# nico-bohlinger/RL-X

Measured on NVIDIA H100. Metric: env-steps/sec (PPO update incl.), higher is better.
Workload: dtype f32

## Files before the change

### rl_x_b200/csrc/gemm_tc.cu

```cuda
#include "gemm_dispatch.cuh"
#include "gemm_tc_common.cuh"

namespace rlx {
namespace tc {

struct Cfg {
  static constexpr int A_BYTES = BM * BK * 4;
  static constexpr int B_BYTES = BN * BK * 4;
  static constexpr int RAW_BYTES = A_BYTES + B_BYTES;
  static constexpr int OP_BYTES = 2 * B_BYTES;
  static constexpr int RAW_STAGES = 3, OP_STAGES = 4;
  static constexpr int SMEM_BYTES = RAW_STAGES * RAW_BYTES + OP_STAGES * OP_BYTES + 1024  + 1024 ;
  static constexpr int SPLIT_STAGE_BYTES = A_BYTES + 2 * B_BYTES;
  static constexpr int SPLIT_STAGES = 4;
  static constexpr int SPLIT_SMEM_BYTES = SPLIT_STAGES * SPLIT_STAGE_BYTES + 1024 + 1024;
  static constexpr int PRODUCER_REGS = 56, CONSUMER_REGS = 224;
};
static_assert(Cfg::SMEM_BYTES <= 227 * 1024 && Cfg::SPLIT_SMEM_BYTES <= 227 * 1024, "shared memory of one H100 block");
static_assert(Cfg::PRODUCER_REGS * 128 + Cfg::CONSUMER_REGS * 256 <= 65536, "register file of one SM");

template <bool KMAJ, bool BF16, int ROWS>
__device__ __forceinline__ void convert_tile(const uint8_t* raw, uint8_t* hi, uint8_t* lo, int t) {
  constexpr uint32_t HI = 0xFFFFE000u;
  if (KMAJ) {
// ... 178 lines not shown

  if (warp < 4) {
    setmaxnreg_dec<Cfg::PRODUCER_REGS>();
    const int t = threadIdx.x;
    uint64_t* ld_empty = SPLIT_B ? op_empty : raw_empty;
    int ld_tile = blockIdx.x, ld_kb = 0, ld_count = 0;
    auto load_next = [&]() {
      while (ld_tile < num_tiles) {
        int zb, zs, m0, n0, kbeg, nkb;
        tile_coords(ld_tile, zb, zs, m0, n0, kbeg, nkb);
        if (ld_kb >= nkb) {
          ld_tile += gridDim.x;
          ld_kb = 0;
          continue;
        }
        const int slot = ld_count % RAW_STAGES;
        mbar_wait(&ld_empty[slot], ((ld_count / RAW_STAGES) & 1) ^ 1);
        uint8_t* sa = smem + slot * RAW_BYTES;
        uint8_t* sb = sa + Cfg::A_BYTES;
        uint64_t* bar = &raw_full[slot];
        const int k0 = kbeg + ld_kb * BK;
        mbar_arrive_expect_tx(bar, RAW_BYTES);
        if (A_KMAJ) {
          tma_load_2d(&tmap_a, bar, sa, p.a_k_off * zb + k0, p.a_mn_off * zb + m0);
        } else {
#pragma unroll
          for (int j = 0; j < BM / 32; ++j) tma_load_2d(&tmap_a, bar, sa + j * (BK * 128), p.a_mn_off * zb + m0 + 32 * j, p.a_k_off * zb + k0);
        }
        if (B_KMAJ) {
          tma_load_2d(&tmap_b, bar, sb, p.b_k_off * zb + k0, p.b_mn_off * zb + n0);
          if (SPLIT_B) tma_load_2d(&tmap_b_lo, bar, sb + Cfg::B_BYTES, p.b_k_off * zb + k0, p.b_mn_off * zb + n0);
        } else {
#pragma unroll
          for (int j = 0; j < BN / 32; ++j) tma_load_2d(&tmap_b, bar, sb + j * (BK * 128), p.b_mn_off * zb + n0 + 32 * j, p.b_k_off * zb + k0);
        }
        ++ld_kb;
        ++ld_count;
        return true;
      }
      return false;
    };
    if constexpr (SPLIT_B) {
      if (t == 0)
        while (load_next()) {
        }
      return;
    }
    if (t == 0)
      for (int i = 0; i < RAW_STAGES; ++i) load_next();
    int rs = 0, os = 0;
    uint32_t rph = 0, oph = 0;
    bool refill = false;
    for (int tile = blockIdx.x; tile < num_tiles; tile += gridDim.x) {
      int zb, zs, m0, n0, kbeg, nkb;
      tile_coords(tile, zb, zs, m0, n0, kbeg, nkb);
      for (int kb = 0; kb < nkb; ++kb) {
        mbar_wait(&raw_full[rs], rph);
        mbar_wait(&op_empty[os], oph ^ 1);
        uint8_t* op = ops + os * Cfg::OP_BYTES;
        convert_tile<B_KMAJ, BF16, BN>(smem + rs * Cfg::RAW_BYTES + Cfg::A_BYTES, op, op + Cfg::B_BYTES, t);
        fence_proxy_async();
        named_bar_sync(1, 128);
        if (t == 0) {
          mbar_arrive(&op_full[os]);
          mbar_arrive(&raw_empty[rs]);
          if (refill) load_next();
          refill = true;
        }
        if (++rs == RAW_STAGES) { rs = 0; rph ^= 1; }
        if (++os == OP_STAGES) { os = 0; oph ^= 1; }
      }
    }
  } else {
    setmaxnreg_inc<Cfg::CONSUMER_REGS>();
    const int cw = (warp >> 2) - 1;
    const int r0 = cw * 64 + (warp & 3) * 16 + (lane >> 2);
    float acc[64], cor[64];
    uint32_t ah[2][2][4], al[2][2][4];
    int rs = 0, os = 0;
    uint32_t rph = 0, oph = 0;
    for (int tile = blockIdx.x; tile < num_tiles; tile += gridDim.x) {
      int zb, zs, m0, n0, kbeg, nkb;
      tile_coords(tile, zb, zs, m0, n0, kbeg, nkb);
      for (int kb = 0; kb < nkb; ++kb) {
        mbar_wait(&raw_full[rs], rph);
        if (!SPLIT_B) mbar_wait(&op_full[os], oph);
        const uint8_t* raw = smem + rs * RAW_BYTES;
        const uint32_t op = SPLIT_B ? smem_u32(raw + Cfg::A_BYTES) : smem_u32(ops + os * Cfg::OP_BYTES);
        const uint64_t db = make_smem_desc(op), db_lo = make_smem_desc(op + Cfg::B_BYTES);
#pragma unroll
        for (int h = 0; h < 2; ++h) {
          load_a_frags<A_KMAJ, BF16>(raw, r0, lane, h, ah[h], al[h]);
          if (!SPLIT_B && h == 1) {
            __syncwarp();
            if (lane == 0) mbar_arrive(&raw_empty[rs]);
          }
          fence_frags(ah[h]);
          if (!BF16) fence_frags(al[h]);
          wgmma_fence();
#pragma unroll
          for (int q = 0; q < 2; ++q) {
            const int kk = 2 * h + q;
            const uint64_t ko = (uint64_t)((kk * WG_K * 4) >> 4);
            const uint32_t accum = (kb | kk) != 0 ? 1u : 0u;
            if (!BF16) {
              wgmma_tf32_m64n128k8(cor, al[h][q], db + ko, accum);
              wgmma_tf32_m64n128k8(cor, ah[h][q], db_lo + ko, 1u);
            }
            wgmma_tf32_m64n128k8(acc, ah[h][q], db + ko, accum);
          }
          wgmma_commit();
          wgmma_wait_1();
          if (h == 0 && kb > 0 && lane == 0) mbar_arrive(&op_empty[os == 0 ? OP_STAGES - 1 : os - 1]);
        }
        if (++rs == RAW_STAGES) { rs = 0; rph ^= 1; }
        if (++os == OP_STAGES) { os = 0; oph ^= 1; }
      }

      constexpr bool HAS_AUX = (EPI == TC_EPI_DTANH || EPI == TC_EPI_DRELU);
      constexpr bool HAS_BIAS = (EPI == TC_EPI_BIAS_TANH || EPI == TC_EPI_BIAS_RELU || EPI == TC_EPI_BIAS);
      const int m = m0 + r0, ct = n0 + 2 * (lane & 3);
      const bool full = m0 + BM <= (TRANS ? p.m_main : p.M) && n0 + BN <= p.N;
      const int clim = p.N - 1 - ct;
      const float* abase = HAS_AUX ? p.aux + p.aux_batch_off * zb + ct : nullptr;
      float e[2][32];
      auto load_aux = [&](int q) {
        const float* arow = abase + (long long)min(m + 8 * (q >> 1), p.M - 1) * p.ldaux;
        if (full) load_cols<true>(e[q >> 1], arow, clim, 8 * (q & 1));
        else load_cols<false>(e[q >> 1], arow, clim, 8 * (q & 1));
      };
      if (HAS_BIAS) {
        const float* b = p.bias + p.bias_batch_off * zb + ct;
#pragma unroll
        for (int c0 = 0; c0 < 16; c0 += 8) {
          if (full) load_cols<true>(e[0], b, clim, c0);
          else load_cols<false>(e[0], b, clim, c0);
        }
      }
      if (HAS_AUX) load_aux(0);
      if (nkb > 0) {
        wgmma_wait_all();
        if (lane == 0) mbar_arrive(&op_empty[os == 0 ? OP_STAGES - 1 : os - 1]);
      }
      fence_acc(acc);
      if (!BF16) fence_acc(cor);
      float* cbase = p.C + p.c_batch_off * zb + p.c_split_off * zs;
      float* ebase = (TRANS && p.extra_row != nullptr) ? p.extra_row + p.extra_batch_off * zb + p.extra_split_off * zs : nullptr;
      if (full) store_tile<EPI, BF16, TRANS, true>(acc, cor, e, p, cbase, ebase, m, ct, load_aux);
      else store_tile<EPI, BF16, TRANS, false>(acc, cor, e, p, cbase, ebase, m, ct, load_aux);
    }
  }
}

template <bool A_KMAJ, bool B_KMAJ, int EPI, bool BF16 = false, bool TRANS = false, bool SPLIT_B = false>
static int launch_cfg(const TcOperand& A, const TcOperand& B, TcParams p, int kclass, cudaStream_t stream, const float* b_lo = nullptr) {
  CUtensorMap ta, tb, tb_lo;
  int rc = make_tmap(&ta, A.base, A.rows, A.cols, A.ld, 32, A_KMAJ ? BM : BK);
  if (rc) return rc;
  rc = make_tmap(&tb, B.base, B.rows, B.cols, B.ld, 32, B_KMAJ ? BN : BK);
  if (rc) return rc;
  if (SPLIT_B) {
    rc = make_tmap(&tb_lo, b_lo, B.rows, B.cols, B.ld, 32, BN);
    if (rc) return rc;
  } else {
    tb_lo = tb;
  }
// ... 167 lines not shown
```

### rl_x_b200/csrc/gemm_tc_common.cuh

```cuda
#pragma once
#include <cuda.h>

#include "common.cuh"
#include "gemm_simt.cuh"

namespace rlx {
namespace tc {

constexpr int BM = 128;
constexpr int BN = 128;
constexpr int BK = 32;
constexpr int WG_K = 8;
constexpr int NUM_THREADS = 384;

enum TcEpi { TC_EPI_NONE = 0, TC_EPI_BIAS_TANH = 1, TC_EPI_DTANH = 2, TC_EPI_BIAS_RELU = 3, TC_EPI_DRELU = 4, TC_EPI_BIAS = 5 };

struct TcParams {
  int M, N, K;
  int batch, splits, kchunk;
  int tiles_m, tiles_n;
  int a_mn_off, a_k_off, b_mn_off, b_k_off;
  float* C;
  long long ldc, c_batch_off, c_split_off;
  int m_main;
  float* extra_row;
  long long extra_batch_off, extra_split_off;
  const float* bias;
  long long bias_batch_off;
  const float* aux;
  long long ldaux, aux_batch_off;
  int single;
  int bf16;
};

__device__ __forceinline__ uint32_t smem_u32(const void* p) { return (uint32_t)__cvta_generic_to_shared(p); }

__device__ __forceinline__ void mbar_init(uint64_t* bar, uint32_t count) {
  asm volatile("mbarrier.init.shared::cta.b64 [%0], %1;" ::"r"(smem_u32(bar)), "r"(count) : "memory");
}
__device__ __forceinline__ void mbar_wait(uint64_t* bar, uint32_t parity) {
  asm volatile(
      "{\n\t"
      ".reg .pred P1;\n\t"
      "WAIT_LOOP:\n\t"
      "mbarrier.try_wait.parity.shared::cta.b64 P1, [%0], %1;\n\t"
      "@P1 bra WAIT_DONE;\n\t"
      "bra WAIT_LOOP;\n\t"
      "WAIT_DONE:\n\t"
      "}" ::"r"(smem_u32(bar)), "r"(parity)
      : "memory");
}
__device__ __forceinline__ void mbar_arrive(uint64_t* bar) {
  asm volatile("mbarrier.arrive.shared::cta.b64 _, [%0];" ::"r"(smem_u32(bar)) : "memory");
}
__device__ __forceinline__ void mbar_arrive_expect_tx(uint64_t* bar, uint32_t bytes) {
  asm volatile("mbarrier.arrive.expect_tx.shared::cta.b64 _, [%0], %1;" ::"r"(smem_u32(bar)), "r"(bytes) : "memory");
}
__device__ __forceinline__ void fence_barrier_init() { asm volatile("fence.mbarrier_init.release.cluster;" ::: "memory"); }
__device__ __forceinline__ void fence_proxy_async() { asm volatile("fence.proxy.async.shared::cta;" ::: "memory"); }
__device__ __forceinline__ void named_bar_sync(int id, int threads) { asm volatile("bar.sync %0, %1;" ::"r"(id), "r"(threads) : "memory"); }

__device__ __forceinline__ void tma_load_2d(const CUtensorMap* map, uint64_t* bar, void* smem, int c0, int c1) {
  asm volatile("cp.async.bulk.tensor.2d.shared::cluster.global.mbarrier::complete_tx::bytes [%0], [%1, {%3, %4}], [%2];" ::"r"(smem_u32(smem)),
               "l"((uint64_t)map), "r"(smem_u32(bar)), "r"(c0), "r"(c1)
               : "memory");
}
__device__ __forceinline__ void prefetch_tmap(const CUtensorMap* map) {
  asm volatile("prefetch.tensormap [%0];" ::"l"((uint64_t)map) : "memory");
}

__device__ __forceinline__ uint64_t make_smem_desc(uint32_t saddr) {
  uint64_t d = 0;
  d |= (uint64_t)((saddr >> 4) & 0x3FFFu);
  d |= (uint64_t)1u << 16;
  d |= (uint64_t)(1024u >> 4) << 32;
  d |= 1ull << 62;
  return d;
}

__device__ __forceinline__ void wgmma_fence() { asm volatile("wgmma.fence.sync.aligned;" ::: "memory"); }
__device__ __forceinline__ void wgmma_commit() { asm volatile("wgmma.commit_group.sync.aligned;" ::: "memory"); }
__device__ __forceinline__ void wgmma_wait_all() { asm volatile("wgmma.wait_group.sync.aligned 0;" ::: "memory"); }
__device__ __forceinline__ void wgmma_wait_1() { asm volatile("wgmma.wait_group.sync.aligned 1;" ::: "memory"); }
__device__ __forceinline__ void fence_acc(float (&d)[64]) {
#pragma unroll
  for (int i = 0; i < 64; ++i) asm volatile("" : "+f"(d[i])::"memory");
}
__device__ __forceinline__ void fence_frags(uint32_t (&a)[2][4]) {
#pragma unroll
  for (int i = 0; i < 2; ++i)
#pragma unroll
    for (int j = 0; j < 4; ++j) asm volatile("" : "+r"(a[i][j])::"memory");
}

template <int N> __device__ __forceinline__ void setmaxnreg_dec() { asm volatile("setmaxnreg.dec.sync.aligned.u32 %0;" ::"n"(N)); }
template <int N> __device__ __forceinline__ void setmaxnreg_inc() { asm volatile("setmaxnreg.inc.sync.aligned.u32 %0;" ::"n"(N)); }

__device__ __forceinline__ void wgmma_tf32_m64n128k8(float (&d)[64], const uint32_t (&a)[4], uint64_t b_desc, uint32_t accumulate) {
  asm volatile(
      "{\n\t"
      ".reg .pred p;\n\t"
      "setp.ne.b32 p, %69, 0;\n\t"
      "wgmma.mma_async.sync.aligned.m64n128k8.f32.tf32.tf32 "
      "{%0, %1, %2, %3, %4, %5, %6, %7, %8, %9, %10, %11, %12, %13, %14, %15, "
      "%16, %17, %18, %19, %20, %21, %22, %23, %24, %25, %26, %27, %28, %29, %30, %31, "
      "%32, %33, %34, %35, %36, %37, %38, %39, %40, %41, %42, %43, %44, %45, %46, %47, "
      "%48, %49, %50, %51, %52, %53, %54, %55, %56, %57, %58, %59, %60, %61, %62, %63}, "
      "{%64, %65, %66, %67}, %68, p, 1, 1;\n\t"
      "}"
      : "+f"(d[0]), "+f"(d[1]), "+f"(d[2]), "+f"(d[3]), "+f"(d[4]), "+f"(d[5]), "+f"(d[6]), "+f"(d[7]), "+f"(d[8]), "+f"(d[9]),
        "+f"(d[10]), "+f"(d[11]), "+f"(d[12]), "+f"(d[13]), "+f"(d[14]), "+f"(d[15]), "+f"(d[16]), "+f"(d[17]), "+f"(d[18]),
        "+f"(d[19]), "+f"(d[20]), "+f"(d[21]), "+f"(d[22]), "+f"(d[23]), "+f"(d[24]), "+f"(d[25]), "+f"(d[26]), "+f"(d[27]),
        "+f"(d[28]), "+f"(d[29]), "+f"(d[30]), "+f"(d[31]), "+f"(d[32]), "+f"(d[33]), "+f"(d[34]), "+f"(d[35]), "+f"(d[36]),
        "+f"(d[37]), "+f"(d[38]), "+f"(d[39]), "+f"(d[40]), "+f"(d[41]), "+f"(d[42]), "+f"(d[43]), "+f"(d[44]), "+f"(d[45]),
        "+f"(d[46]), "+f"(d[47]), "+f"(d[48]), "+f"(d[49]), "+f"(d[50]), "+f"(d[51]), "+f"(d[52]), "+f"(d[53]), "+f"(d[54]),
        "+f"(d[55]), "+f"(d[56]), "+f"(d[57]), "+f"(d[58]), "+f"(d[59]), "+f"(d[60]), "+f"(d[61]), "+f"(d[62]), "+f"(d[63])
      : "r"(a[0]), "r"(a[1]), "r"(a[2]), "r"(a[3]), "l"(b_desc), "r"(accumulate)
      : "memory");
}


typedef CUresult (*EncodeTiledFn)(CUtensorMap*, CUtensorMapDataType, cuuint32_t, void*, const cuuint64_t*, const cuuint64_t*, const cuuint32_t*,
                                  const cuuint32_t*, CUtensorMapInterleave, CUtensorMapSwizzle, CUtensorMapL2promotion, CUtensorMapFloatOOBfill);

static inline EncodeTiledFn get_encode_fn() {
  static EncodeTiledFn fn = nullptr;
  static bool tried = false;
  if (!tried) {
    tried = true;
    void* ptr = nullptr;
    cudaDriverEntryPointQueryResult q;
    if (cudaGetDriverEntryPoint("cuTensorMapEncodeTiled", &ptr, cudaEnableDefault, &q) == cudaSuccess && q == cudaDriverEntryPointSuccess)
      fn = reinterpret_cast<EncodeTiledFn>(ptr);
  }
  return fn;
}

static inline int make_tmap(CUtensorMap* map, const float* base, long long rows, long long cols, long long ld, int box_cols, int box_rows) {
  EncodeTiledFn fn = get_encode_fn();
  if (!fn) {
    set_error("tensor-core engine: cuTensorMapEncodeTiled is unavailable");
    return RLX_ERR_UNSUPPORTED;
  }
  cuuint64_t gdim[2] = {(cuuint64_t)cols, (cuuint64_t)rows};
  cuuint64_t gstride[1] = {(cuuint64_t)ld * 4};
  cuuint32_t box[2] = {(cuuint32_t)box_cols, (cuuint32_t)box_rows};
  cuuint32_t estr[2] = {1, 1};
// ... 18 lines not shown
```

### rl_x_b200/csrc/ppo.cu

```cuda
#include "common.cuh"
#include "gemm_simt.cuh"
#include "gemm_dispatch.cuh"
#include "ppo_head.cuh"
#include "ppo_head_gemm.cuh"
#include "ppo_head_mma.cuh"
#include "ppo_optim.cuh"

namespace rlx {

static bool use_tc(const rlx_ppo_dims& d) { return g_gemm_engine == 1 && tc_supported(d); }
}
int comm_allreduce_ppo(rlx_comm* c, float* out, int64_t n, const rlx_ppo_dims& d, float* norm_partials, long long* step_count, void* stream, int* nblk_out);
namespace rlx {

struct Splits {
  int splits, kchunk;
};
static Splits choose_splits(long long rows, int out_m, int out_n, int batch, bool tc) {
  if (tc) {
    const long long tiles = ceil_div(out_m, 128) * ceil_div(out_n, 128) * batch;
    const long long smin = std::max<long long>(1, ceil_div(rows, 1024)), smax = std::max<long long>(smin, std::min<long long>(smin + 64, rows / 64));
    const long long sms = sm_count();
    long long best = smin;
    double best_fill = -1.0;
// ... 262 lines not shown
}

static long long tall_elements(const GradReduceP& r) {
  long long tall = 0;
  for (int gi = 0; gi < kNumGroups; ++gi)
    if (r.g[gi].nsplit > kTallSplit) tall += r.g[gi].len;
  return tall;
}
static double partial_bytes(const GradReduceP& r) {
  double b = 0;
  for (int gi = 0; gi < kNumGroups; ++gi) b += 4.0 * r.g[gi].nsplit * r.g[gi].len;
  return b;
}
static int launch_grad_reduce(const GradReduceP& r, cudaStream_t st) {
  const int flat_blocks = (int)ceil_div(r.total, 256);
  const int tall_blocks = (int)ceil_div(tall_elements(r), 8);
  RLX_LAUNCH_C(KC_GRAD_REDUCE, 0, partial_bytes(r) + 4.0 * r.total, ppo_grad_reduce_kernel, (unsigned)(flat_blocks + tall_blocks), 256, 0, st, r, flat_blocks);
  return RLX_OK;
}

static bool fast_head_ok(const PpoLayout& L) { return (L.act <= 31) && (L.H % 2 == 0) && (L.H <= 1024); }

static int launch_train_head(const rlx_ppo_minibatch_args* a, const PpoLayout& L, const TrainPlan& P, const float* params, int bf16, cudaStream_t st) {
  const long long m = a->m;
  const int H = L.H, A = L.act;
  void* ws = a->workspace;
  float* H2 = ws_ptr<float>(ws, P.off_H2);
  float* dZ2 = ws_ptr<float>(ws, P.off_dZ2);
  float* dhead = ws_ptr<float>(ws, P.off_dhead);
  float* headpart = ws_ptr<float>(ws, P.off_headpart);
  const float inv_mg = 1.f / (float)a->m_global;
  HeadP h{};
  fill_head_common(h, L, params, H2, m);
  h.bf16 = bf16;
  h.actions = a->actions; h.logp_old = a->log_probs; h.adv = a->advantages; h.ret = a->returns; h.adv_stats = a->adv_stats;
  h.inv_mg = inv_mg; h.clip_range = a->hp.clip_range; h.critic_coef = a->hp.critic_coef;
  h.ratio_delta_metric = a->hp.ratio_delta_metric != 0.f ? 1 : 0;
  const bool want_median = a->hp.ratio_delta_metric == 2.f;
  h.ratio_abs = want_median ? ws_ptr<float>(ws, P.off_ratio) : nullptr;
  h.dZ2 = dZ2; h.dhead = dhead; h.block_partials = headpart;
  int head_blocks = P.head_blocks;
  const size_t smem = head_smem_bytes(a->dims, true);
  const int dh_ld = (int)(ceil_div(A + 1, 4) * 4);
  const bool fast_head = fast_head_ok(L);
  const double head_flops = 4.0 * m * H * (A + 1), head_bytes = 4.0 * m * (4.0 * H + 2.0 * A + 5);
  const bool gemm_head = fast_head && g_head_engine == 1 && !bf16 && head_gemm_scratch_floats(m, H, A) <= m * 2LL * H;
  if (gemm_head) {
    HeadGemmArgs ha{m, H, A, dh_ld, H2, a->params + L.off[W3P], a->params + L.off[W3C], a->params + L.off[B3P], a->params + L.off[B3C],
                    a->params + L.off[LOGSTD], a->actions, a->log_probs, a->advantages, a->returns, a->adv_stats, inv_mg, a->hp.clip_range,
                    a->hp.critic_coef, a->hp.ratio_delta_metric != 0.f ? 1 : 0, dZ2, dhead, headpart, ws_ptr<float>(ws, P.off_dZ1)};
    const int rc = ppo_head_gemm_path(ha, st);
    if (rc) return rc;
    return 1;
  }
  if (!fast_head) {
    RLX_DISPATCH_NCH(KC_HEAD_TRAIN, head_flops, head_bytes, H, ppo_head_train_kernel, head_blocks, 256, smem, st, h);
    return head_blocks;
  }
  HeadTrain2Extra ex{dh_ld};
  const bool vec_head = (H == 128 || H == 256 || H == 512);
  const int nt4 = (int)ceil_div(dh_ld, 8);
  const size_t smem4 = head4_smem_floats(H, A, nt4) * sizeof(float);
  const bool mma_head = vec_head && g_head_engine == 2 && !bf16 && nt4 <= 4 && smem4 <= 220 * 1024;
  if (mma_head) {
    head_blocks = (int)std::min<long long>(ceil_div(m, 16 * kHead4RowTiles), (long long)P.head_blocks);
#define RLX_HEAD4(H_, NT_)                                                                                                          \
  do {                                                                                                                              \
    RLX_CHECK_CUDA(cudaFuncSetAttribute(ppo_head_train4_kernel<H_, NT_>, cudaFuncAttributeMaxDynamicSharedMemorySize, (int)smem4)); \
    RLX_LAUNCH_C(KC_HEAD_TRAIN, head_flops, head_bytes, (ppo_head_train4_kernel<H_, NT_>), head_blocks, 256, smem4, st, h, ex);     \
  } while (0)
#define RLX_HEAD4_NT(H_)              \
  do {                                \
    if (nt4 == 1) RLX_HEAD4(H_, 1);   \
    else if (nt4 == 2) RLX_HEAD4(H_, 2); \
    else if (nt4 == 3) RLX_HEAD4(H_, 3); \
    else RLX_HEAD4(H_, 4);            \
  } while (0)
    if (H == 128) RLX_HEAD4_NT(128);
    else if (H == 256) RLX_HEAD4_NT(256);
    else RLX_HEAD4_NT(512);
#undef RLX_HEAD4_NT
#undef RLX_HEAD4
  } else if (vec_head) {
#define RLX_HEAD3_B(H_, AM_, BF_)                                                                                                     \
  do {                                                                                                                                \
    RLX_CHECK_CUDA(cudaFuncSetAttribute(ppo_head_train3_kernel<H_, AM_, BF_>, cudaFuncAttributeMaxDynamicSharedMemorySize, (int)smem)); \
    RLX_LAUNCH_C(KC_HEAD_TRAIN, head_flops, head_bytes, (ppo_head_train3_kernel<H_, AM_, BF_>), head_blocks, 256, smem, st, h, ex);    \
  } while (0)
#define RLX_HEAD3(H_, AM_)                          \
  do {                                              \
    if (bf16) RLX_HEAD3_B(H_, AM_, true);           \
    else RLX_HEAD3_B(H_, AM_, false);               \
  } while (0)
#define RLX_HEAD3_ACT(H_)                      \
  do {                                         \
    if (A <= 8) RLX_HEAD3(H_, 8);              \
    else if (A <= 16) RLX_HEAD3(H_, 16);       \
    else if (A <= 24) RLX_HEAD3(H_, 24);       \
    else RLX_HEAD3(H_, 31);                    \
  } while (0)
    if (H == 128) RLX_HEAD3_ACT(128);
    else if (H == 256) RLX_HEAD3_ACT(256);
    else RLX_HEAD3_ACT(512);
#undef RLX_HEAD3_ACT
#undef RLX_HEAD3
#undef RLX_HEAD3_B
  } else {
    const int nch = (int)ceil_div(H, 32);
#define RLX_HEAD2_B(NCH_, AM_, BF_)                                                                                                   \
  do {                                                                                                                                \
    RLX_CHECK_CUDA(cudaFuncSetAttribute(ppo_head_train2_kernel<NCH_, AM_, BF_>, cudaFuncAttributeMaxDynamicSharedMemorySize, (int)smem)); \
    RLX_LAUNCH_C(KC_HEAD_TRAIN, head_flops, head_bytes, (ppo_head_train2_kernel<NCH_, AM_, BF_>), head_blocks, 256, smem, st, h, ex);  \
  } while (0)
#define RLX_HEAD2(NCH_, AM_)                        \
  do {                                              \
    if (bf16) RLX_HEAD2_B(NCH_, AM_, true);         \
    else RLX_HEAD2_B(NCH_, AM_, false);             \
  } while (0)
#define RLX_HEAD2_ACT(NCH_)                         \
  do {                                              \
    if (A <= 8) RLX_HEAD2(NCH_, 8);                 \
    else if (A <= 16) RLX_HEAD2(NCH_, 16);          \
    else if (A <= 24) RLX_HEAD2(NCH_, 24);          \
    else RLX_HEAD2(NCH_, 31);                       \
  } while (0)
    if (nch <= 2) RLX_HEAD2_ACT(2);
    else if (nch <= 4) RLX_HEAD2_ACT(4);
    else if (nch <= 8) RLX_HEAD2_ACT(8);
    else if (nch <= 16) RLX_HEAD2_ACT(16);
    else RLX_HEAD2_ACT(32);
#undef RLX_HEAD2_ACT
#undef RLX_HEAD2
#undef RLX_HEAD2_B
  }
  return head_blocks;
}

struct W3Partials {
  float* src;
  int nsplit;
  long long stride, critic_off;
};
static W3Partials chunked_w3(const PpoLayout& L, float* part3, int nchunks) {
  return W3Partials{part3, nchunks, (long long)(L.act + 1) * L.H, (long long)L.act * L.H};
}

static int launch_head_wgrad(const PpoLayout& L, const TrainPlan& P, long long m, bool tc, int bf16, void* ws, cudaStream_t st, W3Partials& w3) {
  const int H = L.H, A = L.act;
  float* H2 = ws_ptr<float>(ws, P.off_H2);
  float* dhead = ws_ptr<float>(ws, P.off_dhead);
  float* part3 = ws_ptr<float>(ws, P.off_part3);
  const int wgrad_chunks = (int)ceil_div(m, kHeadWgradRows);
  const double wflops = 2.0 * m * H * (A + 1), wbytes = 4.0 * m * (2.0 * H + A + 1);
  if (!fast_head_ok(L)) {
    HeadWgradP w{(int)m, H, A, kHeadWgradRows, H2, dhead, part3};
    dim3 wg((unsigned)wgrad_chunks, (unsigned)ceil_div(2 * H, 256));
    const size_t wsmem = (size_t)kHeadWgradRows * (A + 1) * sizeof(float);
    if (A <= 8) RLX_LAUNCH_C(KC_HEAD_WGRAD, wflops, wbytes, ppo_head_wgrad_kernel<8>, wg, 256, wsmem, st, w);
    else if (A <= 32) RLX_LAUNCH_C(KC_HEAD_WGRAD, wflops, wbytes, ppo_head_wgrad_kernel<32>, wg, 256, wsmem, st, w);
    else {
      RLX_CHECK_CUDA(cudaFuncSetAttribute(ppo_head_wgrad_kernel<64>, cudaFuncAttributeMaxDynamicSharedMemorySize, (int)wsmem));
      RLX_LAUNCH_C(KC_HEAD_WGRAD, wflops, wbytes, ppo_head_wgrad_kernel<64>, wg, 256, wsmem, st, w);
    }
    count_gemm_path(GP_HEAD_WGRAD_SIMT);
    w3 = chunked_w3(L, part3, wgrad_chunks);
    return RLX_OK;
  }
  const int dh_ld = (int)(ceil_div(A + 1, 4) * 4);
  if (tc) {
    const Splits S3 = choose_splits(m, dh_ld, H, 2, true);
// ... 352 lines not shown
```

### rl_x_b200/csrc/ppo_head.cuh

```cuda
#pragma once
#include "common.cuh"

namespace rlx {

constexpr float kLogSqrt2Pi = 0.91893853320467274178f;

__device__ __forceinline__ void philox4x32_10(uint32_t (&c)[4], uint32_t k0, uint32_t k1) {
#pragma unroll
  for (int r = 0; r < 10; ++r) {
    const uint32_t hi0 = __umulhi(0xD2511F53u, c[0]), lo0 = 0xD2511F53u * c[0];
    const uint32_t hi1 = __umulhi(0xCD9E8D57u, c[2]), lo1 = 0xCD9E8D57u * c[2];
    const uint32_t n0 = hi1 ^ c[1] ^ k0, n1 = lo1, n2 = hi0 ^ c[3] ^ k1, n3 = lo0;
    c[0] = n0; c[1] = n1; c[2] = n2; c[3] = n3;
    k0 += 0x9E3779B9u; k1 += 0xBB67AE85u;
  }
}
__device__ __forceinline__ float philox_normal(uint64_t seed, uint64_t offset, uint32_t row, uint32_t j) {
  uint32_t c[4] = {row, j >> 2, (uint32_t)offset, (uint32_t)(offset >> 32)};
  philox4x32_10(c, (uint32_t)seed, (uint32_t)(seed >> 32));
  const uint32_t a = (j & 2) ? c[2] : c[0], b = (j & 2) ? c[3] : c[1];
  const float u1 = ((float)a + 0.5f) * 2.3283064365386963e-10f;
  const float u2 = ((float)b + 0.5f) * 2.3283064365386963e-10f;
  const float r = sqrtf(-2.f * logf(fminf(u1, 1.f)));
  float s, co;
  sincospif(2.f * u2, &s, &co);
  return (j & 1) ? r * s : r * co;
}

struct HeadP {
  int M, H, act;
  const float* H2;
  const float* W3p;
  const float* W3c;
  const float* b3p;
  const float* b3c;
  const float* logstd;
  const float* noise;
  unsigned long long seed, offset;
  const float* act_low;
  const float* act_high;
  int clip_rescale, deterministic;
  float* action;
  float* env_action;
  float* logp_out;
  float* value_out;
  const float* actions;
  const float* logp_old;
  const float* adv;
  const float* ret;
  const float* adv_stats;
  float inv_mg;
  float clip_range, critic_coef;
  int ratio_delta_metric;
  float* ratio_abs;
  float* dZ2;
  float* dhead;
  float* block_partials;
  int bf16;
};

template <int NCH, bool BF16>
__device__ __forceinline__ void head_row_forward(const HeadP& p, const float* __restrict__ sW3p, const float* __restrict__ sW3c,
                                                 long long row, int lane, float (&hp)[NCH], float (&hc)[NCH], float& mean_lo,
                                                 float& mean_hi, float& value) {
  const float* __restrict__ h = p.H2 + row * (2LL * p.H);
#pragma unroll
  for (int c = 0; c < NCH; ++c) {
    const int j = lane + 32 * c;
    hp[c] = (j < p.H) ? h[j] : 0.f;
    hc[c] = (j < p.H) ? h[p.H + j] : 0.f;
  }
  mean_lo = 0.f;
  mean_hi = 0.f;
  for (int a = 0; a < p.act; ++a) {
    float s = 0.f;
#pragma unroll
    for (int c = 0; c < NCH; ++c) {
      const int j = lane + 32 * c;
      if (j < p.H) s = fmaf(hp[c], sW3p[a * p.H + j], s);
    }
    s = bf16r_if(warp_sum(s) + p.b3p[a], BF16);
    if (lane == (a & 31)) {
      if (a < 32) mean_lo = s; else mean_hi = s;
    }
// ... 343 lines not shown
#pragma unroll
    for (int c = 0; c < NCH; ++c) dz0[c] = dz1[c] = 0.f;
#pragma unroll
    for (int a = 0; a < ACT_MAX; ++a) {
      if (a < act) {
        const float g0 = __shfl_sync(0xffffffffu, dmean[0], a);
        const float g1 = __shfl_sync(0xffffffffu, dmean[1], a);
#pragma unroll
        for (int c = 0; c < NCH; ++c) {
          const int j = lane + 32 * c;
          const float w = (j < H) ? sW3p[a * H + j] : 0.f;
          dz0[c] = fmaf(g0, w, dz0[c]);
          dz1[c] = fmaf(g1, w, dz1[c]);
        }
      }
    }
#pragma unroll
    for (int r = 0; r < 2; ++r) {
      if (r == 1 && !has1) break;
      float* __restrict__ out = p.dZ2 + (row0 + r) * (2LL * H);
#pragma unroll
      for (int c = 0; c < NCH; ++c) {
        const int j = lane + 32 * c;
        if (j < H) {
          const float hpv = hp[r][c], hcv = hc[r][c];
          const float zp = bf16r_if(bf16r_if(r ? dz1[c] : dz0[c], BF16) * (1.f - hpv * hpv), BF16);
          const float zc = bf16r_if(bf16r_if(dvv[r] * sW3c[j], BF16) * (1.f - hcv * hcv), BF16);
          out[j] = zp;
          out[H + j] = zc;
          acc_db2p[c] += zp;
          acc_db2c[c] += zc;
        }
      }
    }
  }

  float* my = sred + wib * npart;
  if (own) {
    my[lane] = acc_db3;
    my[act + 1 + lane] = acc_dls;
  } else if (lane == act) {
    my[act] = acc_db3;
  }
  if (lane == 0) {
    my[2 * act + 1] = acc_pg;
    my[2 * act + 2] = acc_vl;
    my[2 * act + 3] = acc_kl;
    my[2 * act + 4] = acc_cf;
  }
#pragma unroll
  for (int c = 0; c < NCH; ++c) {
    const int j = lane + 32 * c;
    if (j < H) {
      my[2 * act + 5 + j] = acc_db2p[c];
      my[2 * act + 5 + H + j] = acc_db2c[c];
    }
  }
  __syncthreads();
  for (int i = threadIdx.x; i < npart; i += blockDim.x) {
    float s = 0.f;
    for (int w = 0; w < nw; ++w) s += sred[w * npart + i];
    p.block_partials[(long long)blockIdx.x * npart + i] = s;
  }
}

struct HeadWgrad2P {
  int M, H, act, dh_ld, rows_per_chunk;
  const float* H2;
  const float* dhead;
  float* part;
};

__device__ __forceinline__ float dot4(const float4& a, const float4& b, float s) {
  s = fmaf(a.x, b.x, s); s = fmaf(a.y, b.y, s); s = fmaf(a.z, b.z, s); return fmaf(a.w, b.w, s);
}
__device__ __forceinline__ void axpy4(float g, const float4& w, float4& d) {
  d.x = fmaf(g, w.x, d.x); d.y = fmaf(g, w.y, d.y); d.z = fmaf(g, w.z, d.z); d.w = fmaf(g, w.w, d.w);
}

template <int H_, int ACT_MAX, bool BF16 = false>
__global__ void __launch_bounds__(256, 2) ppo_head_train3_kernel(const HeadP p, const HeadTrain2Extra ex) {
  constexpr int NG = H_ / 128;
  constexpr int H4 = H_ / 4;
  extern __shared__ __align__(16) float smem[];
  float* sW3p = smem;
  float* sW3c = smem + p.act * H_;
  float* sred = sW3c + H_;
  head_stage_weights(p, sW3p, sW3c);
  const float4* sW3p4 = reinterpret_cast<const float4*>(sW3p);
  const float4* sW3c4 = reinterpret_cast<const float4*>(sW3c);
  const int lane = threadIdx.x & 31, wib = threadIdx.x >> 5, nw = blockDim.x >> 5;
  const int act = p.act;
  const int npart = 2 * act + 5 + 2 * H_;
  const float adv_mean = p.adv_stats[0];
  const float adv_den = p.adv_stats[1] + 1e-8f;
  const float clip_lo = 1.f - p.clip_range, clip_hi = 1.f + p.clip_range;
  const bool own = lane < act;
  const float my_b3 = own ? p.b3p[lane] : ((lane == act) ? p.b3c[0] : 0.f);
  const float my_sd = own ? expf(p.logstd[lane]) : 1.f;
  const float my_var = my_sd * my_sd;
  const float my_logsd = logf(my_sd);

  float4 acc_db2p[NG], acc_db2c[NG];
#pragma unroll
  for (int g = 0; g < NG; ++g) acc_db2p[g] = acc_db2c[g] = make_float4(0.f, 0.f, 0.f, 0.f);
  float acc_db3 = 0.f, acc_dls = 0.f, acc_pg = 0.f, acc_vl = 0.f, acc_kl = 0.f, acc_cf = 0.f;

  const long long npairs = ((long long)p.M + 1) / 2;
  for (long long pr = (long long)blockIdx.x * nw + wib; pr < npairs; pr += (long long)gridDim.x * nw) {
    const long long row0 = 2 * pr;
    const bool has1 = row0 + 1 < p.M;
    float4 hp[2][NG], hc[2][NG];
#pragma unroll
    for (int r = 0; r < 2; ++r) {
      const float4* __restrict__ h = reinterpret_cast<const float4*>(p.H2 + (row0 + ((r == 1 && !has1) ? 0 : r)) * (2LL * H_));
#pragma unroll
      for (int g = 0; g < NG; ++g) {
        hp[r][g] = h[g * 32 + lane];
        hc[r][g] = h[H4 + g * 32 + lane];
      }
    }
    float v0[32], v1[32];
#pragma unroll
    for (int a = 0; a < 32; ++a) v0[a] = v1[a] = 0.f;
#pragma unroll
    for (int a = 0; a < ACT_MAX; ++a) {
      if (a < act) {
        float s0 = 0.f, s1 = 0.f;
#pragma unroll
        for (int g = 0; g < NG; ++g) {
          const float4 w = sW3p4[a * H4 + g * 32 + lane];
          s0 = dot4(hp[0][g], w, s0);
          s1 = dot4(hp[1][g], w, s1);
        }
        v0[a] = s0;
        v1[a] = s1;
      }
    }
    {
      float s0 = 0.f, s1 = 0.f;
#pragma unroll
      for (int g = 0; g < NG; ++g) {
        const float4 w = sW3c4[g * 32 + lane];
        s0 = dot4(hc[0][g], w, s0);
        s1 = dot4(hc[1][g], w, s1);
      }
#pragma unroll
      for (int a = 0; a < 32; ++a)
        if (a == act) { v0[a] = s0; v1[a] = s1; }
    }
    const float out0 = bf16r_if(butterfly_reduce32(v0, lane) + my_b3, BF16);
    const float out1 = bf16r_if(butterfly_reduce32(v1, lane) + my_b3, BF16);

    float dmean[2], dvv[2];
#pragma unroll
    for (int r = 0; r < 2; ++r) {
      const long long row = row0 + r;
      const bool valid = (r == 0) || has1;
      const float out = r ? out1 : out0;
      const float value = __shfl_sync(0xffffffffu, out, act);
      float lp = 0.f, dmu = 0.f, zz = 0.f;
      if (own && valid) {
        const float d = p.actions[row * act + lane] - out;
        lp = -(d * d) / (2.f * my_var) - my_logsd - kLogSqrt2Pi;
        dmu = d / my_var;
        zz = d * d / my_var;
      }
      const float logp_new = warp_sum(lp);
      float dm = 0.f, dv = 0.f;
      if (valid) {
        const float logratio = logp_new - p.logp_old[row];
        const float ratio = expf(logratio);
        const float A = (p.adv[row] - adv_mean) / adv_den;
        const float pg1 = -A * ratio;
        const float pg2 = -A * fminf(fmaxf(ratio, clip_lo), clip_hi);
        const float w1 = (pg1 > pg2) ? 1.f : ((pg1 == pg2) ? 0.5f : 0.f);
        const float inr = (ratio >= clip_lo && ratio <= clip_hi) ? 1.f : 0.f;
        const float dlogp = (-A * (w1 + (1.f - w1) * inr)) * ratio * p.inv_mg;
        const float verr = value - p.ret[row];
        dv = bf16r_if(p.critic_coef * verr * p.inv_mg, BF16);
        acc_pg += fmaxf(pg1, pg2);
        acc_vl += 0.5f * verr * verr;
        acc_kl += (ratio - 1.f) - logratio;
        acc_cf += p.ratio_delta_metric ? fabsf(ratio - 1.f) : ((fabsf(ratio - 1.f) > p.clip_range) ? 1.f : 0.f);
        if (p.ratio_abs != nullptr && lane == 0) p.ratio_abs[row] = fabsf(ratio - 1.f);
        dm = bf16r_if(dlogp * dmu, BF16);
        if (own) {
          acc_db3 += dm;
          acc_dls += dlogp * (zz - 1.f);
          p.dhead[row * ex.dh_ld + lane] = dm;
        } else if (lane == act) {
          acc_db3 += dv;
          p.dhead[row * ex.dh_ld + act] = dv;
        } else if (lane < ex.dh_ld) {
          p.dhead[row * ex.dh_ld + lane] = 0.f;
        }
      }
      dmean[r] = dm;
      dvv[r] = dv;
    }
    float4 dz0[NG], dz1[NG];
#pragma unroll
    for (int g = 0; g < NG; ++g) dz0[g] = dz1[g] = make_float4(0.f, 0.f, 0.f, 0.f);
#pragma unroll
    for (int a = 0; a < ACT_MAX; ++a) {
      if (a < act) {
        const float g0 = __shfl_sync(0xffffffffu, dmean[0], a);
        const float g1 = __shfl_sync(0xffffffffu, dmean[1], a);
#pragma unroll
        for (int g = 0; g < NG; ++g) {
          const float4 w = sW3p4[a * H4 + g * 32 + lane];
          axpy4(g0, w, dz0[g]);
          axpy4(g1, w, dz1[g]);
        }
      }
    }
#pragma unroll
    for (int r = 0; r < 2; ++r) {
      if (r == 1 && !has1) break;
      float4* __restrict__ out = reinterpret_cast<float4*>(p.dZ2 + (row0 + r) * (2LL * H_));
#pragma unroll
      for (int g = 0; g < NG; ++g) {
        const float4 a4 = hp[r][g], c4 = hc[r][g], d4 = r ? dz1[g] : dz0[g], wc = sW3c4[g * 32 + lane];
        float4 zp, zc;
        constexpr int bf = BF16 ? 1 : 0;
        zp.x = bf16r_if(bf16r_if(d4.x, bf) * (1.f - a4.x * a4.x), bf); zp.y = bf16r_if(bf16r_if(d4.y, bf) * (1.f - a4.y * a4.y), bf);
        zp.z = bf16r_if(bf16r_if(d4.z, bf) * (1.f - a4.z * a4.z), bf); zp.w = bf16r_if(bf16r_if(d4.w, bf) * (1.f - a4.w * a4.w), bf);
        zc.x = bf16r_if(bf16r_if(dvv[r] * wc.x, bf) * (1.f - c4.x * c4.x), bf); zc.y = bf16r_if(bf16r_if(dvv[r] * wc.y, bf) * (1.f - c4.y * c4.y), bf);
        zc.z = bf16r_if(bf16r_if(dvv[r] * wc.z, bf) * (1.f - c4.z * c4.z), bf); zc.w = bf16r_if(bf16r_if(dvv[r] * wc.w, bf) * (1.f - c4.w * c4.w), bf);
        out[g * 32 + lane] = zp;
        out[H4 + g * 32 + lane] = zc;
        acc_db2p[g].x += zp.x; acc_db2p[g].y += zp.y; acc_db2p[g].z += zp.z; acc_db2p[g].w += zp.w;
        acc_db2c[g].x += zc.x; acc_db2c[g].y += zc.y; acc_db2c[g].z += zc.z; acc_db2c[g].w += zc.w;
      }
    }
  }

  float* my = sred + wib * npart;
  if (own) {
    my[lane] = acc_db3;
    my[act + 1 + lane] = acc_dls;
  } else if (lane == act) {
    my[act] = acc_db3;
  }
  if (lane == 0) {
    my[2 * act + 1] = acc_pg;
    my[2 * act + 2] = acc_vl;
    my[2 * act + 3] = acc_kl;
    my[2 * act + 4] = acc_cf;
  }
#pragma unroll
  for (int g = 0; g < NG; ++g) {
    float* q = my + 2 * act + 5 + g * 128 + 4 * lane;
    q[0] = acc_db2p[g].x; q[1] = acc_db2p[g].y; q[2] = acc_db2p[g].z; q[3] = acc_db2p[g].w;
    q[H_] = acc_db2c[g].x; q[H_ + 1] = acc_db2c[g].y; q[H_ + 2] = acc_db2c[g].z; q[H_ + 3] = acc_db2c[g].w;
  }
  __syncthreads();
  for (int i = threadIdx.x; i < npart; i += blockDim.x) {
    float s = 0.f;
    for (int w = 0; w < nw; ++w) s += sred[w * npart + i];
    p.block_partials[(long long)blockIdx.x * npart + i] = s;
  }
// ... 103 lines not shown
```

Baseline: 3.375 million.

## Prefetch head activations via bulk async copies and skip empty GEMM consumer tiles

The PPO head training kernel now double-buffers each warp's next row pair of hidden activations into a per-warp shared-memory slot using cp.async.bulk with an mbarrier. It also hoists the per-row scalar loads (actions, old log-prob, advantage, return) ahead of compute, with the aim of hiding global-memory latency behind the dot products. Separately, TC GEMM consumer warpgroups whose 64-row slice lies entirely past M now only drain the pipeline barriers and skip the MMA work. The cost is more shared memory per block, which may reduce occupancy, and more intricate barrier bookkeeping.

```diff
diff --git a/rl_x_b200/csrc/gemm_tc.cu b/rl_x_b200/csrc/gemm_tc.cu
--- a/rl_x_b200/csrc/gemm_tc.cu
+++ b/rl_x_b200/csrc/gemm_tc.cu
@@ -284,6 +284,19 @@
     for (int tile = blockIdx.x; tile < num_tiles; tile += gridDim.x) {
       int zb, zs, m0, n0, kbeg, nkb;
       tile_coords(tile, zb, zs, m0, n0, kbeg, nkb);
+      if (__shfl_sync(0xffffffffu, (int)(m0 + 64 * cw >= p.M), 0)) {
+        for (int kb = 0; kb < nkb; ++kb) {
+          mbar_wait(&raw_full[rs], rph);
+          if (!SPLIT_B) mbar_wait(&op_full[os], oph);
+          __syncwarp();
+          if (kb > 0 && lane == 0) mbar_arrive(&op_empty[os == 0 ? OP_STAGES - 1 : os - 1]);
+          if (!SPLIT_B && lane == 0) mbar_arrive(&raw_empty[rs]);
+          if (++rs == RAW_STAGES) { rs = 0; rph ^= 1; }
+          if (++os == OP_STAGES) { os = 0; oph ^= 1; }
+        }
+        if (nkb > 0 && lane == 0) mbar_arrive(&op_empty[os == 0 ? OP_STAGES - 1 : os - 1]);
+        continue;
+      }
       for (int kb = 0; kb < nkb; ++kb) {
         mbar_wait(&raw_full[rs], rph);
         if (!SPLIT_B) mbar_wait(&op_full[os], oph);
diff --git a/rl_x_b200/csrc/gemm_tc_common.cuh b/rl_x_b200/csrc/gemm_tc_common.cuh
--- a/rl_x_b200/csrc/gemm_tc_common.cuh
+++ b/rl_x_b200/csrc/gemm_tc_common.cuh
@@ -63,6 +63,11 @@
 __device__ __forceinline__ void tma_load_2d(const CUtensorMap* map, uint64_t* bar, void* smem, int c0, int c1) {
   asm volatile("cp.async.bulk.tensor.2d.shared::cluster.global.mbarrier::complete_tx::bytes [%0], [%1, {%3, %4}], [%2];" ::"r"(smem_u32(smem)),
                "l"((uint64_t)map), "r"(smem_u32(bar)), "r"(c0), "r"(c1)
+               : "memory");
+}
+__device__ __forceinline__ void bulk_load_1d(void* smem, const void* gmem, uint32_t bytes, uint64_t* bar) {
+  asm volatile("cp.async.bulk.shared::cluster.global.mbarrier::complete_tx::bytes [%0], [%1], %2, [%3];" ::"r"(smem_u32(smem)),
+               "l"((uint64_t)gmem), "r"(bytes), "r"(smem_u32(bar))
                : "memory");
 }
 __device__ __forceinline__ void prefetch_tmap(const CUtensorMap* map) {
diff --git a/rl_x_b200/csrc/ppo.cu b/rl_x_b200/csrc/ppo.cu
--- a/rl_x_b200/csrc/ppo.cu
+++ b/rl_x_b200/csrc/ppo.cu
@@ -368,10 +368,13 @@
 #undef RLX_HEAD4_NT
 #undef RLX_HEAD4
   } else if (vec_head) {
-#define RLX_HEAD3_B(H_, AM_, BF_)                                                                                                     \
-  do {                                                                                                                                \
-    RLX_CHECK_CUDA(cudaFuncSetAttribute(ppo_head_train3_kernel<H_, AM_, BF_>, cudaFuncAttributeMaxDynamicSharedMemorySize, (int)smem)); \
-    RLX_LAUNCH_C(KC_HEAD_TRAIN, head_flops, head_bytes, (ppo_head_train3_kernel<H_, AM_, BF_>), head_blocks, 256, smem, st, h, ex);    \
+    const size_t smem3 = smem + 8 * (4 * (size_t)H * sizeof(float) + sizeof(uint64_t));
+#define RLX_HEAD3_B(H_, AM_, BF_)                                                                                                        \
+  do {                                                                                                                                   \
+    RLX_CHECK_CUDA(cudaFuncSetAttribute(ppo_head_train3_kernel<H_, AM_, BF_>, cudaFuncAttributeMaxDynamicSharedMemorySize, (int)smem3));   \
+    RLX_CHECK_CUDA(cudaFuncSetAttribute(ppo_head_train3_kernel<H_, AM_, BF_>, cudaFuncAttributePreferredSharedMemoryCarveout,             \
+                                        cudaSharedmemCarveoutMaxShared));                                                                \
+    RLX_LAUNCH_C(KC_HEAD_TRAIN, head_flops, head_bytes, (ppo_head_train3_kernel<H_, AM_, BF_>), head_blocks, 256, smem3, st, h, ex);      \
   } while (0)
 #define RLX_HEAD3(H_, AM_)                          \
   do {                                              \
diff --git a/rl_x_b200/csrc/ppo_head.cuh b/rl_x_b200/csrc/ppo_head.cuh
--- a/rl_x_b200/csrc/ppo_head.cuh
+++ b/rl_x_b200/csrc/ppo_head.cuh
@@ -1,5 +1,6 @@
 #pragma once
 #include "common.cuh"
+#include "gemm_tc_common.cuh"
 
 namespace rlx {
 
@@ -509,16 +510,32 @@
 __global__ void __launch_bounds__(256, 2) ppo_head_train3_kernel(const HeadP p, const HeadTrain2Extra ex) {
   constexpr int NG = H_ / 128;
   constexpr int H4 = H_ / 4;
+  constexpr int SLOT = 4 * H_;
   extern __shared__ __align__(16) float smem[];
   float* sW3p = smem;
   float* sW3c = smem + p.act * H_;
   float* sred = sW3c + H_;
+  const int lane = threadIdx.x & 31, wib = threadIdx.x >> 5, nw = blockDim.x >> 5;
+  const int act = p.act;
+  const int npart = 2 * act + 5 + 2 * H_;
+  float* slot = sred + nw * npart + wib * SLOT;
+  uint64_t* full = reinterpret_cast<uint64_t*>(sred + nw * npart + nw * SLOT) + wib;
+  const long long npairs = ((long long)p.M + 1) / 2;
+  const long long pstride = (long long)gridDim.x * nw;
+  auto fetch = [&](long long pr) {
+    const long long row0 = 2 * pr;
+    const uint32_t bytes = (row0 + 1 < p.M ? 2u : 1u) * 2u * H_ * sizeof(float);
+    tc::mbar_arrive_expect_tx(full, bytes);
+    tc::bulk_load_1d(slot, p.H2 + row0 * (2LL * H_), bytes, full);
+  };
+  if (lane == 0) {
+    tc::mbar_init(full, 1);
+    tc::fence_barrier_init();
+    if ((long long)blockIdx.x * nw + wib < npairs) fetch((long long)blockIdx.x * nw + wib);
+  }
   head_stage_weights(p, sW3p, sW3c);
   const float4* sW3p4 = reinterpret_cast<const float4*>(sW3p);
   const float4* sW3c4 = reinterpret_cast<const float4*>(sW3c);
-  const int lane = threadIdx.x & 31, wib = threadIdx.x >> 5, nw = blockDim.x >> 5;
-  const int act = p.act;
-  const int npart = 2 * act + 5 + 2 * H_;
   const float adv_mean = p.adv_stats[0];
   const float adv_den = p.adv_stats[1] + 1e-8f;
   const float clip_lo = 1.f - p.clip_range, clip_hi = 1.f + p.clip_range;
@@ -533,19 +550,36 @@
   for (int g = 0; g < NG; ++g) acc_db2p[g] = acc_db2c[g] = make_float4(0.f, 0.f, 0.f, 0.f);
   float acc_db3 = 0.f, acc_dls = 0.f, acc_pg = 0.f, acc_vl = 0.f, acc_kl = 0.f, acc_cf = 0.f;
 
-  const long long npairs = ((long long)p.M + 1) / 2;
-  for (long long pr = (long long)blockIdx.x * nw + wib; pr < npairs; pr += (long long)gridDim.x * nw) {
+  uint32_t phase = 0;
+  for (long long pr = (long long)blockIdx.x * nw + wib; pr < npairs; pr += pstride) {
     const long long row0 = 2 * pr;
     const bool has1 = row0 + 1 < p.M;
     float4 hp[2][NG], hc[2][NG];
+    tc::mbar_wait(full, phase);
+    phase ^= 1;
+    float in_act[2], in_logp[2], in_adv[2], in_ret[2];
 #pragma unroll
     for (int r = 0; r < 2; ++r) {
-      const float4* __restrict__ h = reinterpret_cast<const float4*>(p.H2 + (row0 + ((r == 1 && !has1) ? 0 : r)) * (2LL * H_));
+      const long long row = row0 + r;
+      const bool valid = (r == 0) || has1;
+      in_act[r] = (own && valid) ? p.actions[row * act + lane] : 0.f;
+      in_logp[r] = valid ? p.logp_old[row] : 0.f;
+      in_adv[r] = valid ? p.adv[row] : 0.f;
+      in_ret[r] = valid ? p.ret[row] : 0.f;
+    }
+#pragma unroll
+    for (int r = 0; r < 2; ++r) {
+      const float4* h = reinterpret_cast<const float4*>(slot + ((r == 1 && !has1) ? 0 : r) * 2 * H_);
 #pragma unroll
       for (int g = 0; g < NG; ++g) {
         hp[r][g] = h[g * 32 + lane];
         hc[r][g] = h[H4 + g * 32 + lane];
       }
+    }
+    __syncwarp();
+    if (lane == 0 && pr + pstride < npairs) {
+      tc::fence_proxy_async();
+      fetch(pr + pstride);
     }
     float v0[32], v1[32];
 #pragma unroll
@@ -588,7 +622,7 @@
       const float value = __shfl_sync(0xffffffffu, out, act);
       float lp = 0.f, dmu = 0.f, zz = 0.f;
       if (own && valid) {
-        const float d = p.actions[row * act + lane] - out;
+        const float d = in_act[r] - out;
         lp = -(d * d) / (2.f * my_var) - my_logsd - kLogSqrt2Pi;
         dmu = d / my_var;
         zz = d * d / my_var;
@@ -596,15 +630,15 @@
       const float logp_new = warp_sum(lp);
       float dm = 0.f, dv = 0.f;
       if (valid) {
-        const float logratio = logp_new - p.logp_old[row];
+        const float logratio = logp_new - in_logp[r];
         const float ratio = expf(logratio);
-        const float A = (p.adv[row] - adv_mean) / adv_den;
+        const float A = (in_adv[r] - adv_mean) / adv_den;
         const float pg1 = -A * ratio;
         const float pg2 = -A * fminf(fmaxf(ratio, clip_lo), clip_hi);
         const float w1 = (pg1 > pg2) ? 1.f : ((pg1 == pg2) ? 0.5f : 0.f);
         const float inr = (ratio >= clip_lo && ratio <= clip_hi) ? 1.f : 0.f;
         const float dlogp = (-A * (w1 + (1.f - w1) * inr)) * ratio * p.inv_mg;
-        const float verr = value - p.ret[row];
+        const float verr = value - in_ret[r];
         dv = bf16r_if(p.critic_coef * verr * p.inv_mg, BF16);
         acc_pg += fmaxf(pg1, pg2);
         acc_vl += 0.5f * verr * verr;
```

Result: no change. 3.391 million, median of 6 (+0.5%).
